# ZJU-FAST-Lab/Dftpav

Hardware: AMD Instinct MI355X
Metric: trajectory solves/sec (batched), 16-piece MINCO (higher is better)
Workload: dtype f64

## Files before the change

dftpav_amd/csrc/quad_common.h:

```cpp
#pragma once
#include "ref_order_common.h"

namespace dftpav {
namespace reford {

__device__ __forceinline__ double row_chain16(double acc, double v) {
  const double one = 1.0;
  asm volatile("s_nop 1\n\t" DFTPAV_FMAC_BCAST16 : "+v"(acc) : "v"(v), "v"(one));
  return acc;
}
__device__ __forceinline__ double row_add_lane0(double acc, double v) {
  const double one = 1.0;
  asm volatile("s_nop 1\n\t" DFTPAV_FMAC_BCAST(0) : "+v"(acc) : "v"(v), "v"(one));
  return acc;
}
__device__ __forceinline__ double row_max16(double v) {
  v = fmax(v, mov_dpp<0xB1>(v));
  v = fmax(v, mov_dpp<0x4E>(v));
  v = fmax(v, mov_dpp<0x141>(v));
  v = fmax(v, mov_dpp<0x140>(v));
  return v;
}
template <int CTRL> __device__ __forceinline__ double nb_dpp(double v) {
  int lo = __double2loint(v), hi = __double2hiint(v);
  lo = __builtin_amdgcn_update_dpp(0, lo, CTRL, 0xf, 0xf, true);
  hi = __builtin_amdgcn_update_dpp(0, hi, CTRL, 0xf, 0xf, true);
  return __hiloint2double(hi, lo);
}


constexpr int kQPool = 64;
__host__ __device__ constexpr size_t q4_team_doubles(int mem) { return 32 + 32 + 12 + 6 + sNUM + (size_t)mem + kQPool * 3 + kQPool / 8; }
__host__ __device__ constexpr size_t q4_team_bytes(int mem) { return (q4_team_doubles(mem) * sizeof(double) + iNUM * sizeof(int) + 15) & ~(size_t)15; }
__host__ __device__ constexpr size_t q4_shared_bytes(int N) { return ((size_t)pk_segment_doubles(N) * sizeof(double) + 15) & ~(size_t)15; }
constexpr size_t kDenseEntryBytes = 4 + 8 + 15 * 8;
__host__ __device__ constexpr size_t q4_dense_bytes_of(int k) { return ((size_t)k * kDenseEntryBytes + 15) & ~(size_t)15; }
constexpr int kDenseSizedForN = 16, kDenseSizedForMem = 256;
__host__ __device__ constexpr int q4_dense_capacity(int N, int mem) {
  int k = 64;
  while (k > 8 && 4 * (q4_shared_bytes(N) + 4 * q4_team_bytes(mem) + q4_dense_bytes_of(k)) > (size_t)160 * 1024) k -= 8;
  return k;
}
constexpr int kDense = q4_dense_capacity(kDenseSizedForN, kDenseSizedForMem);
static_assert(kDense % 8 == 0 && kDense >= 8 && kDense <= 64, "a lane's slots of the list are the bits of a 64-bit mask (solver_ref4.hip: mine |= 1ull << e)");
static_assert(4 * (q4_shared_bytes(kDenseSizedForN) + 4 * q4_team_bytes(kDenseSizedForMem) + q4_dense_bytes_of(kDense)) <= (size_t)160 * 1024,
              "four workgroups of one wave share a CU's LDS at 16 pieces and a history of 256");
typedef unsigned long long dmask_t;
struct DenseLds {
  ldsi_t id;
  ldsd_t s1;
  ldsd_t out;
};
__host__ __device__ constexpr size_t q4_dense_bytes() { return q4_dense_bytes_of(kDense); }
__device__ inline void q4_carve_dense(DenseLds &d, char *base) {
  ldsd_t p = (ldsd_t)reinterpret_cast<double *>(base);
  d.s1 = p; p += kDense;
  d.out = p; p += 15 * kDense;
  d.id = (ldsi_t)p;
}

}
}
```

dftpav_amd/csrc/solver_ref4.hip:

```cpp
#include <hip/hip_runtime.h>
#include <cstdio>
#include <cstdlib>
#include <algorithm>

#include "ref_order_common.h"
#include "quad_lbfgs.h"

namespace dftpav {
namespace reford {

static_assert(kQPool <= 64 && kQPool % 8 == 0, "a lane's pool slots are the bits of a 64-bit mask; the chain pass reads the permutation eight bytes at a time");
typedef unsigned char __attribute__((address_space(3))) *ldsb_t;
typedef const unsigned long long __attribute__((address_space(3))) *ldscu64_t;
#ifndef DFTPAV_Q4_WAVES_PER_EU
#define DFTPAV_Q4_WAVES_PER_EU 1
#endif
constexpr int kQ4WavesPerCU = 4 * DFTPAV_Q4_WAVES_PER_EU;

struct Q4 {
  ldsd_t xs, gs;
  ldsd_t bnd;
  ldsd_t tw;
  ldsd_t st;
  ldsd_t alpha;
  ldsd_t pool;
  ldsb_t perm;
  ldsi_t ist;
};
__device__ inline void q4_carve(Q4 &q, char *team, int mem) {
  ldsd_t p = (ldsd_t)reinterpret_cast<double *>(team);
  q.xs = p; p += 32;
  q.gs = p; p += 32;
  q.bnd = p; p += 12;
  q.tw = p; p += 6;
  q.st = p; p += sNUM;
  q.alpha = p; p += mem;
  q.pool = p; p += kQPool * 3;
  q.perm = (ldsb_t)p; p += kQPool / 8;
  q.ist = (ldsi_t)p;
}

__device__ __forceinline__ double row_sum32(double p0, double p1, int n, int l) {
  double acc = row_chain16(0.0, l < n ? p0 : -0.0);
  if (n > 16) acc = row_chain16(acc, 16 + l < n ? p1 : -0.0);
  return acc;
}
template <int Q>
__device__ __forceinline__ void sweep4(ldscd_t tab, double (&bq)[12], int N, int l) {
  constexpr bool DESC = Q == 1 || Q == 3, DIV = Q == 1 || Q == 2;
  ldscd_t ip = tab + 48;
  v2d_t c[pk_size(Q) / 2];
  {
    const int sl = DESC ? N - 1 - l : l;
    const int bi = sl >= 1 && sl <= N - 2 ? sl - 1 : 0;
    const ldscv2_t a = (ldscv2_t)(ip + bi * pk_size(Q));
    if (N > 2) {
#pragma unroll
      for (int u = 0; u < pk_size(Q) / 2; u++) c[u] = a[u];
    } else {
#pragma unroll
      for (int u = 0; u < pk_size(Q) / 2; u++) c[u] = v2d_t{0.0, 0.0};
    }
  }
#pragma unroll 1
  for (int s = 0; s < N; s++) {
    const int p = DESC ? N - 1 - s : s;
    double w[6][2];
#pragma unroll
    for (int r = 0; r < 6; r++)
#pragma unroll
      for (int d = 0; d < 2; d++) {
        w[r][d] = DESC ? nb_dpp<0x101>(bq[2 * (5 - r) + d]) : nb_dpp<0x111>(bq[2 * r + d]);
      }
    if (s == 0 || s == N - 1) {
      const ldscv2_t a = (ldscv2_t)(s == 0 ? tab : ip + (N - 2) * pk_size(Q));
      if (s == 0) {
#pragma unroll
        for (int r = 0; r < 6; r++) w[r][0] = w[r][1] = 0.0;
      }
      if (l == p) {
#pragma unroll
        for (int r = 0; r < 6; r++) {
          v2d_t ce[4];
#pragma unroll
          for (int u = 0; u < 4; u++) ce[u] = a[4 * r + u];
          const int rr = DESC ? 5 - r : r;
#pragma unroll
          for (int d = 0; d < 2; d++) {
            double acc = bq[2 * rr + d];
#pragma unroll
            for (int k = 0; k < 6; k++) {
              const double ck = (k & 1) ? ce[k >> 1].y : ce[k >> 1].x;
              const double t = ck * w[(r + k) % 6][d];
              acc = ck != 0.0 ? acc - t : acc;
            }
            if (DIV) acc = div_by_rcp(acc, ce[3].x, ce[3].y);
            w[r][d] = acc;
            bq[2 * rr + d] = acc;
          }
        }
      }
    } else {
      if (l == p) {
        auto at = [&](int o) { return (o & 1) ? c[o >> 1].y : c[o >> 1].x; };
#pragma unroll
        for (int r = 0; r < 6; r++) {
          const int rr = DESC ? 5 - r : r;
#pragma unroll
          for (int d = 0; d < 2; d++) {
            double acc = bq[2 * rr + d];
#pragma unroll
            for (int k = 0; k < 6; k++)
              if (pk_mask(Q, r) & (1 << k)) acc = acc - at(pk_off(Q, r, k)) * w[(r + k) % 6][d];
            if (DIV) acc = div_by_rcp(acc, at(pk_diag0(Q) + 2 * r), at(pk_diag0(Q) + 2 * r + 1));
            w[r][d] = acc;
            bq[2 * rr + d] = acc;
          }
        }
      }
    }
  }
}

__device__ __forceinline__ void q4_split(const double (&bq)[12], double (&X)[6], double (&Y)[6], int l) {
  const bool lo = (l & 8) == 0;
#pragma unroll
  for (int r = 0; r < 6; r++) {
    const double own = bq[2 * r], far = nb_dpp<0x128>(bq[2 * r + 1]);
    X[r] = lo ? own : far;
    Y[r] = lo ? far : own;
  }
}
__device__ __forceinline__ void q4_unsplit(const double (&X)[6], const double (&Y)[6], double (&bq)[12], int l) {
  const bool lo = (l & 8) == 0;
#pragma unroll
  for (int r = 0; r < 6; r++) {
    bq[2 * r] = lo ? X[r] : Y[r];
    bq[2 * r + 1] = nb_dpp<0x128>(lo ? Y[r] : X[r]);
  }
}
template <int Q>
__device__ __forceinline__ void sweep4_split(ldscd_t tab, double (&X)[6], double (&Y)[6], int l) {
  constexpr bool DESC = Q == 1 || Q == 3, DIV = Q == 1 || Q == 2;
  constexpr int N = 16;
  ldscd_t ip = tab + 48;
  const int l8 = l & 7;
  auto fetch = [&](const double (&R)[6], double (&w)[6]) {
#pragma unroll
    for (int r = 0; r < 6; r++) w[r] = DESC ? nb_dpp<0x101>(R[5 - r]) : nb_dpp<0x111>(R[r]);
  };
  auto end_step = [&](double (&R)[6], double (&w)[6], ldscv2_t a) {
    v2d_t cb[6][4];
#pragma unroll
    for (int r = 0; r < 6; r++)
#pragma unroll
      for (int u = 0; u < (DIV ? 4 : 3); u++) cb[r][u] = a[4 * r + u];
    asm volatile("" ::: "memory");
#pragma unroll
    for (int r = 0; r < 6; r++) {
      const v2d_t(&ce)[4] = cb[r];
      const int rr = DESC ? 5 - r : r;
      double acc = R[rr];
#pragma unroll
      for (int k = 0; k < 6; k++) {
        const double ck = (k & 1) ? ce[k >> 1].y : ce[k >> 1].x;
        const double t = ck * w[(r + k) % 6];
        acc = ck != 0.0 ? acc - t : acc;
      }
      if (DIV) acc = div_by_rcp(acc, ce[3].x, ce[3].y);
      w[r] = acc;
      R[rr] = acc;
    }
  };
  auto interior = [&](double (&R)[6], int s1, double (&w)[6]) {
    v2d_t c[pk_size(Q) / 2];
    {
      const int sl = (s1 & 8) + (DESC ? 7 - l8 : l8);
      const int bi = sl >= 1 && sl <= N - 2 ? sl - 1 : 0;
      const ldscv2_t a = (ldscv2_t)(ip + bi * pk_size(Q));
#pragma unroll
      for (int u = 0; u < pk_size(Q) / 2; u++) c[u] = a[u];
    }
    auto at = [&](int o) { return (o & 1) ? c[o >> 1].y : c[o >> 1].x; };
#pragma unroll 1
    for (int s = s1; s < s1 + 7; s++) {
      const bool own = l8 == ((DESC ? N - 1 - s : s) & 7);
      if (own) {
#pragma unroll
        for (int r = 0; r < 6; r++) {
          const int rr = DESC ? 5 - r : r;
          double acc = R[rr];
#pragma unroll
          for (int k = 0; k < 6; k++)
            if (pk_mask(Q, r) & (1 << k)) acc = acc - at(pk_off(Q, r, k)) * w[(r + k) % 6];
          if (DIV) acc = div_by_rcp(acc, at(pk_diag0(Q) + 2 * r), at(pk_diag0(Q) + 2 * r + 1));
          w[r] = acc;
          R[rr] = acc;
        }
      }
      fetch(R, w);
    }
  };
  double (&A)[6] = DESC ? Y : X;
  double (&B)[6] = DESC ? X : Y;
  double w[6] = {0.0, 0.0, 0.0, 0.0, 0.0, 0.0};
  if (l8 == (DESC ? 7 : 0)) end_step(A, w, (ldscv2_t)tab);
  fetch(A, w);
  interior(A, 1, w);
#pragma unroll
  for (int r = 0; r < 6; r++)
    w[r] = DESC ? nb_dpp<0x12F>(A[5 - r])
                : nb_dpp<0x121>(A[r]);
  interior(B, 8, w);
  if (l8 == (DESC ? 0 : 7)) end_step(B, w, (ldscv2_t)(ip + (N - 2) * pk_size(Q)));
}

struct RectSet {
  d2_t u[5];
};
__device__ __forceinline__ void load_rect(gcd2_t cor, RectSet &r) {
#pragma unroll
  for (int u = 0; u < 5; u++) r.u[u] = cor[16 * u];
}
__device__ __forceinline__ void rect_planes(const RectSet &r, double (&pl)[20]) {
  const double C = r.u[0].x, S = r.u[0].y;
  pl[0] = -S; pl[1] = C;
  pl[4] = C; pl[5] = S;
  pl[8] = S; pl[9] = -C;
  pl[12] = -C; pl[13] = -S;
#pragma unroll
  for (int k = 0; k < 4; k++) {
    pl[4 * k + 2] = r.u[1 + k].x;
    pl[4 * k + 3] = r.u[1 + k].y;
  }
#pragma unroll
  for (int u = 16; u < 20; u++) pl[u] = 0.0;
}
template <bool FAST, bool RECT>
__device__ __forceinline__ double q4_eval(const DevBatch &D, const Q4 &q, const DenseLds &dl, ldscd_t tab, gcd_t cor, size_t cpitch, gd_t ovf, int l, Prof &pr) {
  const DevLayout &L = D.L;
  const DevParams &P = D.P;
  const int N = L.Ntot, H = FAST ? 4 : L.H, nterm = 5 * H + 4, t0 = 5 * H;
  const double epis = FAST ? 0.0 : D.epis;
  const double vt = q.xs[L.x_tau0];
  const double Tr = vt > 0.0 ? ((0.5 * vt + 1.0) * vt + 1.0) + P.mini_T : 1.0 / ((0.5 * vt - 1.0) * vt + 1.0) + P.mini_T;
  const double t1 = Tr / N, t2 = t1 * t1, t3 = t2 * t1, t4 = t2 * t2, t5 = t4 * t1;
  pr.tick(10);
  double bq[12];
#pragma unroll
  for (int u = 0; u < 12; u++) bq[u] = 0.0;
  if (l == 0) {
#pragma unroll
    for (int d = 0; d < 2; d++) {
      bq[0 + d] = q.bnd[d];
      bq[2 + d] = q.bnd[2 + d] * t1;
      bq[4 + d] = q.bnd[4 + d] * t2;
    }
  }
  if (l == N - 1) {
#pragma unroll
    for (int d = 0; d < 2; d++) {
      bq[6 + d] = q.bnd[6 + d];
      bq[8 + d] = q.bnd[8 + d] * t1;
      bq[10 + d] = q.bnd[10 + d] * t2;
    }
  } else if (l < N - 1) {
    bq[10] = q.xs[2 * l];
    bq[11] = q.xs[2 * l + 1];
  }
  if (N == 16) {
    double X[6], Y[6];
    q4_split(bq, X, Y, l);
    sweep4_split<0>(tab, X, Y, l);
    sweep4_split<1>(tab + pk_sweep_offset(1, 16), X, Y, l);
    q4_unsplit(X, Y, bq, l);
  } else {
    sweep4<0>(tab, bq, N, l);
    sweep4<1>(tab + pk_sweep_offset(1, N), bq, N, l);
  }
  pr.tick(0);
  double cc[12];
  {
    const double tI[6] = {1.0 / 1.0, 1.0 / t1, 1.0 / t2, 1.0 / t3, 1.0 / t4, 1.0 / t5};
#pragma unroll
    for (int u = 0; u < 12; u++) cc[u] = bq[u] * tI[u >> 1];
    if (l == 0) {
#pragma unroll
      for (int u = 0; u < 6; u++) q.tw[u] = tI[u];
    }
  }
  double gdC[12], pE, pG;
  {
    const double *c = cc;
    const double t[6] = {1.0, t1, t2, t3, t4, t5};
    const double n33 = c[6] * c[6] + c[7] * c[7], n44 = c[8] * c[8] + c[9] * c[9], n55 = c[10] * c[10] + c[11] * c[11];
    const double d43 = c[8] * c[6] + c[9] * c[7], d53 = c[10] * c[6] + c[11] * c[7], d54 = c[10] * c[8] + c[11] * c[9];
    pE = 36.0 * n33 * t[1] + 144.0 * d43 * t[2] + 192.0 * n44 * t[3] + 240.0 * d53 * t[3] + 720.0 * d54 * t[4] + 720.0 * n55 * t[5];
    pG = 36.0 * n33 + 288.0 * d43 * t[1] + 576.0 * n44 * t[2] + 720.0 * d53 * t[2] + 2880.0 * d54 * t[3] + 3600.0 * n55 * t[4];
#pragma unroll
    for (int d = 0; d < 2; d++) {
      const double c3 = c[6 + d], c4 = c[8 + d], c5 = c[10 + d];
      gdC[10 + d] = 240.0 * c3 * t[3] + 720.0 * c4 * t[4] + 1440.0 * c5 * t[5];
      gdC[8 + d] = 144.0 * c3 * t[2] + 384.0 * c4 * t[3] + 720.0 * c5 * t[4];
      gdC[6 + d] = 72.0 * c3 * t[1] + 144.0 * c4 * t[2] + 240.0 * c5 * t[3];
      gdC[d] = 0.0;
      gdC[2 + d] = 0.0;
      gdC[4 + d] = 0.0;
    }
  }
  pr.tick(1);
  const bool piece = l < N;
  const int Kl = (l == 0 || l == N - 1) ? L.Kd : L.K;
  const int pt0 = l == 0 ? 0 : (L.Kd + 1) + (l - 1) * (L.K + 1);
  const double step = t1 / Kl;
  const int singul_ = L.singuls[0];
  double s1 = 0.0;
  int cnt = 0;
  int rcnt = 0;
  unsigned long long pmask = 0ull;
  const gd_t ovf_l = ovf + (size_t)pt0 * nterm * 3;
  double pl[20];
  RectSet rs;
  const gcd2_t rcor = (gcd2_t)cor;
  if constexpr (RECT) load_rect(rcor, rs);
  else load_planes(cor, cpitch, H, pl);
  __builtin_amdgcn_s_waitcnt(0x0F70);
  auto take = [&](const double (&r12)[12], double e0, double e1, double e2, int slot) {
#pragma unroll
    for (int u = 0; u < 12; u++) gdC[u] += r12[u];
    if (slot < kQPool) {
      ldsd_t e = q.pool + slot * 3;
      e[0] = e0;
      e[1] = e1;
      e[2] = e2;
      pmask |= 1ull << slot;
    } else {
      gd_t e = ovf_l + (size_t)cnt * 3;
      e[0] = e0;
      e[1] = e1;
      e[2] = e2;
    }
    cnt++;
  };
  const int lane64 = (int)(threadIdx.x & 63);
  int listed = 0;
  dmask_t mine = 0ull;
  const unsigned long long here = __builtin_amdgcn_ballot_w64(true);
  const int row_here[4] = {(int)(here & 1ull), (int)((here >> 16) & 1ull), (int)((here >> 32) & 1ull), (int)((here >> 48) & 1ull)};
  const int my_row = lane64 >> 4;
  const int rank = ((my_row > 0 ? row_here[0] : 0) + (my_row > 1 ? row_here[1] : 0) + (my_row > 2 ? row_here[2] : 0)) * 16 + l;
  const int n_here = 16 * (row_here[0] + row_here[1] + row_here[2] + row_here[3]);
  auto scan_here = [&](int c, int &total, int &row_incl) {
    int v = c;
    v += __builtin_amdgcn_update_dpp(0, v, 0x111, 0xf, 0xf, false);
    v += __builtin_amdgcn_update_dpp(0, v, 0x112, 0xf, 0xf, false);
    v += __builtin_amdgcn_update_dpp(0, v, 0x114, 0xf, 0xf, false);
    v += __builtin_amdgcn_update_dpp(0, v, 0x118, 0xf, 0xf, false);
    row_incl = v;
    const int t0_ = row_here[0] ? __builtin_amdgcn_readlane(v, 15) : 0, t1_ = row_here[1] ? __builtin_amdgcn_readlane(v, 31) : 0;
    const int t2_ = row_here[2] ? __builtin_amdgcn_readlane(v, 47) : 0, t3_ = row_here[3] ? __builtin_amdgcn_readlane(v, 63) : 0;
    total = t0_ + t1_ + t2_ + t3_;
    return v + (my_row > 0 ? t0_ : 0) + (my_row > 1 ? t1_ : 0) + (my_row > 2 ? t2_ : 0);
  };
  auto flush = [&]() {
    for (int first = 0; first < listed; first += n_here) {
    const int slot = first + rank;
    const bool work = slot < listed;
    const int id = dl.id[work ? slot : 0];
    const int o = id & 63, t = (id >> 6) & 63, jo = id >> 12;
    double cco[12];
#pragma unroll
    for (int u = 0; u < 12; u++) cco[u] = __shfl(cc[u], o);
    const double t1o = __shfl(t1, o);
    const int lo = o & 15;
    const int Ko = (lo == 0 || lo == N - 1) ? L.Kd : L.K;
    const double stepo = t1o / Ko;
    if (work) {
      const double nopl[20] = {0.0, 0.0, 0.0, 0.0, 0.0, 0.0, 0.0, 0.0, 0.0, 0.0, 0.0, 0.0, 0.0, 0.0, 0.0, 0.0, 0.0, 0.0, 0.0, 0.0};
      PtState ps;
      (void)point_masks<false>(P, cco, lo, N, jo, Ko, stepo, dl.s1[slot], singul_, epis, H, nopl, (gd_t) nullptr, D.sur, 0.0, 0.0, 0, 0.0, ps);
      double r_[16];
      ldsd_t w = dl.out + 15 * slot;
      const double pk[4] = {w[0], w[1], w[2], w[3]};
      point_emit_pf(P, ps, t, H, t0, [&](int, double &on0, double &on1, double &q0, double &q1) { on0 = pk[0]; on1 = pk[1]; q0 = pk[2]; q1 = pk[3]; },
                    (double *)r_);
      const bool corr = t < t0;
#pragma unroll
      for (int u = 0; u < 13; u++) w[u] = r_[u];
      w[13] = corr ? r_[13] : -0.0;
      w[14] = corr ? -0.0 : r_[13];
    }
    }
    __builtin_amdgcn_fence(__ATOMIC_SEQ_CST, "wavefront");
    unsigned rlo = (unsigned)mine, rhi = (unsigned)(mine >> 32);
    rlo |= (unsigned)__builtin_amdgcn_update_dpp(0, (int)rlo, 0x121, 0xf, 0xf, false);
    rhi |= (unsigned)__builtin_amdgcn_update_dpp(0, (int)rhi, 0x121, 0xf, 0xf, false);
    rlo |= (unsigned)__builtin_amdgcn_update_dpp(0, (int)rlo, 0x122, 0xf, 0xf, false);
    rhi |= (unsigned)__builtin_amdgcn_update_dpp(0, (int)rhi, 0x122, 0xf, 0xf, false);
    rlo |= (unsigned)__builtin_amdgcn_update_dpp(0, (int)rlo, 0x124, 0xf, 0xf, false);
    rhi |= (unsigned)__builtin_amdgcn_update_dpp(0, (int)rhi, 0x124, 0xf, 0xf, false);
    rlo |= (unsigned)__builtin_amdgcn_update_dpp(0, (int)rlo, 0x128, 0xf, 0xf, false);
    rhi |= (unsigned)__builtin_amdgcn_update_dpp(0, (int)rhi, 0x128, 0xf, 0xf, false);
    const dmask_t rowm = ((dmask_t)rhi << 32) | rlo;
    for (dmask_t mm = mine; mm;) {
      const int i = __builtin_ctzll(mm);
      mm &= mm - 1;
      ldscd_t w = dl.out + 15 * i;
      double r12[12];
#pragma unroll
      for (int u = 0; u < 12; u++) r12[u] = w[u];
      take(r12, w[12], w[13], w[14], rcnt + __builtin_popcountll(rowm & ((1ull << i) - 1ull)));
    }
    rcnt += __builtin_popcountll(rowm);
    __builtin_amdgcn_fence(__ATOMIC_SEQ_CST, "wavefront");
    listed = 0;
    mine = 0ull;
  };
#pragma unroll 1
  for (int j = 0; j <= L.Kmax + 1; j++) {
    const bool extra = j > L.Kmax;
    unsigned m = 0u;
    PtState pst;
    double nx[20];
    RectSet nr;
    if constexpr (RECT) {
      load_rect(rcor + (size_t)(j < L.Kmax ? j + 1 : L.Kmax) * 80, nr);
      rect_planes(rs, pl);
    } else {
      load_planes(cor + (size_t)(j < L.Kmax ? j + 1 : L.Kmax) * 16, cpitch, H, nx);
    }
    if (piece && j <= Kl && !extra)
      m = (unsigned)point_masks<false>(P, cc, l, N, j, Kl, step, s1, singul_, epis, H, pl, (gd_t) nullptr, D.sur, 0.0, 0.0, 0, 0.0, pst);
    const double s1_pt = s1;
    s1 += step;
    [[maybe_unused]] long long emit_t0 = 0;
    if (D.prof != nullptr) {
#if defined(DFTPAV_PROF_EMIT_CYCLES)
      emit_t0 = clock64();
#elif defined(DFTPAV_PROF_FLUSH_CYCLES)
#else
      const int pc = __builtin_popcount(m);
      int trips = 0;
      while (__builtin_amdgcn_ballot_w64(pc > trips) != 0ull) trips++;
      pr.count(11, trips);
#endif
    }
    auto plane_of = [&](int k, double &on0, double &on1, double &q0, double &q1) {
      on0 = pl[0]; on1 = pl[1]; q0 = pl[2]; q1 = pl[3];
#pragma unroll
      for (int u = 1; u < 5; u++) {
        on0 = k == u ? pl[4 * u] : on0;
        on1 = k == u ? pl[4 * u + 1] : on1;
        q0 = k == u ? pl[4 * u + 2] : q0;
        q1 = k == u ? pl[4 * u + 3] : q1;
      }
    };
    bool in_place = false;
    const int c = __builtin_popcount(m);
    const bool any = __builtin_amdgcn_ballot_w64(c != 0) != 0ull;
    int incl = 0, total = 0, row_incl = 0;
    if (any) incl = scan_here(c, total, row_incl);
    if (listed > 0 && (extra || listed + total > kDense)) {
#ifdef DFTPAV_PROF_FLUSH_CYCLES
      const long long flush_t0 = D.prof != nullptr ? clock64() : 0;
#endif
      flush();
      if (D.prof != nullptr) {
        pr.count(9, 1ll << 32);
#ifdef DFTPAV_PROF_FLUSH_CYCLES
        pr.count(11, clock64() - flush_t0);
#endif
      }
    }
    if (any && total > kDense) {
      in_place = true;
    } else if (any) {
      int e = listed + incl - c;
      for (unsigned mm = m; mm;) {
        const int t = __builtin_ctz(mm);
        mm &= mm - 1;
        dl.id[e] = lane64 | (t << 6) | (j << 12);
        dl.s1[e] = s1_pt;
        if (t < t0) {
          int v = 0;
#pragma unroll
          for (int qv = 1; qv < 5; qv++) v += t >= qv * H ? 1 : 0;
          double on0, on1, q0, q1;
          plane_of(t - v * H, on0, on1, q0, q1);
          ldsd_t w = dl.out + 15 * e;
          w[0] = on0;
          w[1] = on1;
          w[2] = q0;
          w[3] = q1;
        }
        mine |= 1ull << e;
        e++;
      }
      listed += total;
    }
    if (in_place) {
      int slot = rcnt + row_incl - c;
      rcnt += __builtin_amdgcn_update_dpp(0, row_incl, 0x15F, 0xf, 0xf, false);
      for (unsigned mm = m; mm;) {
        const int t = __builtin_ctz(mm);
        mm &= mm - 1;
        double r_[16];
        point_emit_pf(P, pst, t, H, t0, plane_of, (double *)r_);
        const bool corr = t < t0;
        double r12[12];
#pragma unroll
        for (int u = 0; u < 12; u++) r12[u] = r_[u];
        take(r12, r_[12], corr ? r_[13] : -0.0, corr ? -0.0 : r_[13], slot++);
      }
    }
#ifdef DFTPAV_PROF_EMIT_CYCLES
    if (D.prof != nullptr) pr.count(11, clock64() - emit_t0);
#endif
    if constexpr (RECT) {
      rs = nr;
    } else {
#pragma unroll
      for (int u = 0; u < 20; u++) pl[u] = nx[u];
    }
  }
  __threadfence_block();
  pr.tick(2);
  double gdT = row_chain16(0.0, piece ? pG : -0.0);
  const double en = row_chain16(0.0, piece ? pE : -0.0);
  double cost0 = 0.0, cost2 = 0.0;
  {
    const int pc = piece ? cnt : 0;
    int incl = pc;
    incl += __builtin_amdgcn_update_dpp(0, incl, 0x111, 0xf, 0xf, false);
    incl += __builtin_amdgcn_update_dpp(0, incl, 0x112, 0xf, 0xf, false);
    incl += __builtin_amdgcn_update_dpp(0, incl, 0x114, 0xf, 0xf, false);
    incl += __builtin_amdgcn_update_dpp(0, incl, 0x118, 0xf, 0xf, false);
    const int total = __builtin_amdgcn_update_dpp(0, incl, 0x15F, 0xf, 0xf, false);
    pr.count(9, total);
    int kmax = 0;
#pragma unroll
    for (int r = 0; r < 4; r++)
      if (row_here[r]) kmax = max(kmax, __builtin_amdgcn_readlane(incl, 16 * r + 15));
    const bool slow = kmax > kQPool;
    if (D.prof != nullptr) pr.count(11, slow ? 1ll << 32 : 0ll);
    if (kmax > 0 && !slow) {
      {
        int at = incl - pc;
        for (unsigned long long mm = pmask; mm;) {
          q.perm[at++] = (unsigned char)__builtin_ctzll(mm);
          mm &= mm - 1;
        }
      }
      __builtin_amdgcn_fence(__ATOMIC_SEQ_CST, "wavefront");
      for (int k0 = 0; k0 < kmax; k0 += 8) {
        const unsigned long long pb = *(ldscu64_t)(q.perm + k0);
        double e[8][3];
#pragma unroll
        for (int u = 0; u < 8; u++) {
          const int sl = k0 + u < total ? (int)((pb >> (8 * u)) & 255ull) : 0;
#pragma unroll
          for (int w = 0; w < 3; w++) e[u][w] = q.pool[sl * 3 + w];
        }
#pragma unroll
        for (int u = 0; u < 8; u++) {
          const bool in = k0 + u < total;
          gdT += in ? e[u][0] : -0.0;
          cost0 += in ? e[u][1] : -0.0;
          cost2 += in ? e[u][2] : -0.0;
        }
      }
    } else if (slow) {
      for (int p = 0; p < N; p++) {
        const int src = (lane64 & 48) | p;
        const int c = __shfl(pc, src);
        if (__builtin_amdgcn_ballot_w64(c != 0) == 0ull) continue;
        const unsigned long long pm = ((unsigned long long)(unsigned)__shfl((int)(pmask >> 32), src) << 32) | (unsigned)__shfl((int)pmask, src);
        for (unsigned long long mm = pm; mm;) {
          ldscd_t e = q.pool + __builtin_ctzll(mm) * 3;
          mm &= mm - 1;
          gdT += e[0];
          cost0 += e[1];
          cost2 += e[2];
        }
        const int pp0 = p == 0 ? 0 : (L.Kd + 1) + (p - 1) * (L.K + 1);
        const gcd_t og = (gcd_t)(ovf + (size_t)pp0 * nterm * 3);
        for (int i0 = __builtin_popcountll(pm); i0 < c; i0 += 8) {
          double e[8][3];
#pragma unroll
          for (int u = 0; u < 8; u++) {
            const int i = i0 + u < c ? i0 + u : c - 1;
#pragma unroll
            for (int w = 0; w < 3; w++) e[u][w] = og[(size_t)i * 3 + w];
          }
#pragma unroll
          for (int u = 0; u < 8; u++) {
            if (i0 + u < c) {
              gdT += e[u][0];
              cost0 += e[u][1];
              cost2 += e[u][2];
            }
          }
        }
      }
    }
  }
  pr.tick(3);
  double pA;
  double tI[6];
#pragma unroll
  for (int u = 0; u < 6; u++) tI[u] = q.tw[u];
  {
    const double gdtInv[6] = {0.0, -1.0 * tI[2], -2.0 * tI[3], -3.0 * tI[4], -4.0 * tI[5], -5.0 * tI[5] * tI[1]};
    double acc = 0.0;
#pragma unroll
    for (int k = 0; k < 6; k++) {
      const double gdcol = gdC[2 * k] * bq[2 * k] + gdC[2 * k + 1] * bq[2 * k + 1];
      acc += gdtInv[k] * gdcol;
    }
    pA = acc;
  }
  double adj[12];
#pragma unroll
  for (int u = 0; u < 12; u++) adj[u] = gdC[u] * tI[u >> 1];
  if (N == 16) {
    double X[6], Y[6];
    q4_split(adj, X, Y, l);
    sweep4_split<2>(tab + pk_sweep_offset(2, 16), X, Y, l);
    sweep4_split<3>(tab + pk_sweep_offset(3, 16), X, Y, l);
    q4_unsplit(X, Y, adj, l);
  } else {
    sweep4<2>(tab + pk_sweep_offset(2, N), adj, N, l);
    sweep4<3>(tab + pk_sweep_offset(3, N), adj, N, l);
  }
  pr.tick(4);
  if (l < N - 1) {
    q.gs[2 * l] = adj[10];
    q.gs[2 * l + 1] = adj[11];
  }
  {
    double hv[6], tv[6];
#pragma unroll
    for (int u = 0; u < 6; u++) {
      hv[u] = q.bnd[u];
      tv[u] = q.bnd[6 + u];
    }
    const double h1 = hv[2] * adj[2] + hv[3] * adj[3];
    const double h2 = (hv[4] * adj[4] + hv[5] * adj[5]) * 2.0 * t1;
    const double g1 = tv[2] * adj[8] + tv[3] * adj[9];
    const double g2 = (tv[4] * adj[10] + tv[5] * adj[11]) * 2.0 * t1;
    gdT = row_add_lane0(gdT, h1);
    gdT = row_add_lane0(gdT, h2);
    gdT = row_chain16(gdT, l == N - 1 ? g1 : -0.0);
    gdT = row_chain16(gdT, l == N - 1 ? g2 : -0.0);
    gdT = row_chain16(gdT, piece ? pA : -0.0);
    double gdVT2Rt;
    if (vt > 0) {
      gdVT2Rt = vt + 1.0;
    } else {
      const double denSqrt = (0.5 * vt - 1.0) * vt + 1.0;
      gdVT2Rt = (1.0 - vt) / (denSqrt * denSqrt);
    }
    if (l == 0) q.gs[L.x_tau0] = (gdT / N + P.wei_time) * gdVT2Rt;
  }
  double total_smcost = 0.0, total_timecost = 0.0, penalty_cost = 0.0;
  total_smcost += en;
  penalty_cost += (cost0 + 0.0) + cost2;
  total_timecost += Tr * P.wei_time;
  __builtin_amdgcn_fence(__ATOMIC_SEQ_CST, "wavefront");
  pr.tick(5);
  return total_smcost + total_timecost + penalty_cost;
}


constexpr int kQB = 8;
constexpr int kQNpad = 64;
static_assert(kQuadMirrorRows == 2 * kQB, "DevBatch::histM holds kQB rows of either end of a ring");
template <bool Y3> struct QBlk {
  d2_t a[kQB], b[kQB];
  d2_t yr[Y3 ? kQB : 1];
};
typedef double __attribute__((ext_vector_type(2))) qd2_t;

#define DFTPAV_FMAC_BCAST15 \
  DFTPAV_FMAC_BCAST(0) DFTPAV_FMAC_BCAST(1) DFTPAV_FMAC_BCAST(2) DFTPAV_FMAC_BCAST(3) DFTPAV_FMAC_BCAST(4) DFTPAV_FMAC_BCAST(5) DFTPAV_FMAC_BCAST(6) \
  DFTPAV_FMAC_BCAST(7) DFTPAV_FMAC_BCAST(8) DFTPAV_FMAC_BCAST(9) DFTPAV_FMAC_BCAST(10) DFTPAV_FMAC_BCAST(11) DFTPAV_FMAC_BCAST(12) \
  DFTPAV_FMAC_BCAST(13) DFTPAV_FMAC_BCAST(14)
__device__ __forceinline__ double row_chain15(double acc, double v) {
  const double one = 1.0;
  asm volatile("s_nop 1\n\t" DFTPAV_FMAC_BCAST15 : "+v"(acc) : "v"(v), "v"(one));
  return acc;
}
template <bool Y3> __device__ __forceinline__ double q4_rec_sum(double p0, double p1, int n) {
  double acc = row_chain16(0.0, p0);
  if (n > 16) acc = Y3 ? row_chain16(acc, p1) : row_chain15(acc, p1);
  return acc;
}

template <int DIR, bool Y3>
__device__ __forceinline__ void q4_load_blk(QBlk<Y3> &R, gcd2_t hS, gcd2_t hM, gcd2_t hR, int m, int l, int &jl) {
  const bool wrap = DIR < 0 ? jl < kQB - 1 : jl > m - kQB;
  const int mr = DIR < 0 ? kQB + jl : jl - (m - kQB);
  const gcd2_t row = (wrap ? hM + mr * kQNpad : hS + jl * kQNpad) + l;
#pragma unroll
  for (int u = 0; u < kQB; u++) {
    R.a[u] = row[DIR * u * kQNpad];
    R.b[u] = row[DIR * u * kQNpad + 16];
  }
  if (Y3) {
    int jr = jl;
#pragma unroll
    for (int u = 0; u < kQB; u++) {
      R.yr[Y3 ? u : 0] = hR[jr];
      if (DIR < 0) jr = jr == 0 ? m - 1 : jr - 1;
      else jr = jr == m - 1 ? 0 : jr + 1;
    }
  }
  if (DIR < 0) {
    jl -= kQB;
    jl = jl < 0 ? jl + m : jl;
  } else {
    jl += kQB;
    jl = jl >= m ? jl - m : jl;
  }
}
template <bool Y3> __device__ __forceinline__ void q4_pin_blk(QBlk<Y3> &R) {
#pragma unroll
  for (int u = 0; u < kQB; u++) {
    asm volatile("" : "+v"(R.a[u].x), "+v"(R.a[u].y), "+v"(R.b[u].x), "+v"(R.b[u].y));
    if (Y3) asm volatile("" : "+v"(R.yr[Y3 ? u : 0].x), "+v"(R.yr[Y3 ? u : 0].y));
  }
}
template <bool Y3> __device__ __forceinline__ d2_t q4_blk_yr(const QBlk<Y3> &R, int u) {
  if (Y3) return R.yr[Y3 ? u : 0];
  d2_t yr;
  yr.x = mov_dpp<0x15F>(R.b[u].x);
  yr.y = mov_dpp<0x15F>(R.b[u].y);
  return yr;
}
template <bool EXACT, bool Y3>
__device__ __forceinline__ void q4_first_steps(const QBlk<Y3> &R, ldsd_t al, int i0, int bound, int n, int l, bool exact, double &d0, double &d1) {
#pragma unroll
  for (int u = 0; u < kQB; u++) {
    if (i0 + u < bound) {
      const d2_t yr = q4_blk_yr<Y3>(R, u);
      const double dot = q4_rec_sum<Y3>(R.a[u].x * d0, R.b[u].x * d1, n);
      const double a = EXACT && exact ? dot / yr.x : div_by_rcp<false>(dot, yr.x, yr.y);
      if (l == 0) al[u] = a;
      const double na = -a;
      d0 = d0 + na * R.a[u].y;
      d1 = d1 + na * R.b[u].y;
    }
  }
}
template <bool EXACT, bool Y3>
__device__ __forceinline__ void q4_second_steps(const QBlk<Y3> &R, ldscd_t al, int i0, int bound, int n, int l, bool exact, double &d0, double &d1) {
#pragma unroll
  for (int u = 0; u < kQB; u++) {
    if (i0 + u < bound) {
      const double av = al[kQB - 1 - u];
      const d2_t yr = q4_blk_yr<Y3>(R, u);
      const double dot = q4_rec_sum<Y3>(R.a[u].y * d0, R.b[u].y * d1, n);
      const double beta = EXACT && exact ? dot / yr.x : div_by_rcp<false>(dot, yr.x, yr.y);
      const double cf = av - beta;
      d0 = d0 + cf * R.a[u].x;
      d1 = d1 + cf * R.b[u].x;
    }
  }
}
template <bool EXACT, bool Y3>
__device__ __forceinline__ void q4_two_loop(const Q4 &q, gcd2_t hS, gcd2_t hM, gcd2_t hR, int m, int n, int l, int bound, int ne, bool exact, double sc0, double &d0,
                                            double &d1) {
  QBlk<Y3> A, B;
  int jl = ne == 0 ? m - 1 : ne - 1;
  q4_load_blk<-1>(A, hS, hM, hR, m, l, jl);
#pragma unroll 1
  for (int i0 = 0; i0 < bound; i0 += 2 * kQB) {
    q4_pin_blk(A);
    q4_load_blk<-1>(B, hS, hM, hR, m, l, jl);
    q4_first_steps<EXACT>(A, q.alpha + i0, i0, bound, n, l, exact, d0, d1);
    q4_pin_blk(B);
    q4_load_blk<-1>(A, hS, hM, hR, m, l, jl);
    q4_first_steps<EXACT>(B, q.alpha + (i0 + kQB), i0 + kQB, bound, n, l, exact, d0, d1);
  }
  d0 = d0 * sc0;
  d1 = d1 * sc0;
  __builtin_amdgcn_fence(__ATOMIC_SEQ_CST, "wavefront");
  jl = ne - bound;
  jl = jl < 0 ? jl + m : jl;
  q4_load_blk<+1>(A, hS, hM, hR, m, l, jl);
#pragma unroll 1
  for (int i0 = 0; i0 < bound; i0 += 2 * kQB) {
    const ldscd_t al = (ldscd_t)(q.alpha + (bound - kQB - i0));
    q4_pin_blk(A);
    q4_load_blk<+1>(B, hS, hM, hR, m, l, jl);
    q4_second_steps<EXACT>(A, al, i0, bound, n, l, exact, d0, d1);
    q4_pin_blk(B);
    q4_load_blk<+1>(A, hS, hM, hR, m, l, jl);
    q4_second_steps<EXACT>(B, al - kQB, i0 + kQB, bound, n, l, exact, d0, d1);
  }
}
__device__ __forceinline__ void q4_store_pair(gd_t hS, gd_t hM, int m, int end, int e, d2_t v) {
  ((gd2_t)hS)[(size_t)end * kQNpad + e] = v;
  if (end < kQB) ((gd2_t)hM)[(kQB + end) * kQNpad + e] = v;
  if (end >= m - kQB) ((gd2_t)hM)[(end - (m - kQB)) * kQNpad + e] = v;
}

struct Q4Shape {
  static constexpr int NV = 2;
  typedef Q4 Row;
  gd_t hS, hM, hR;
  __device__ __forceinline__ double row_sum(const double (&p)[2], int n, int l) const { return row_sum32(p[0], p[1], n, l); }
  __device__ __forceinline__ void store_pair(int m, int end, int e, d2_t sy) const { q4_store_pair(hS, hM, m, end, e, sy); }
  __device__ __forceinline__ void store_ys(int m, int end, int n, int l, d2_t yr) const {
    if (l == 0) ((gd2_t)hR)[end] = yr;
    if (l == 15 && n <= 31) q4_store_pair(hS, hM, m, end, 31, yr);
  }
  template <bool EXACT>
  __device__ __forceinline__ void two_loop(const Q4 &q, int m, int n, int l, int bound, int ne, bool exact, double sc0, double (&d)[2]) const {
    const gcd2_t cS = (gcd2_t)hS, cM = (gcd2_t)hM, cR = (gcd2_t)hR;
    if (n > 31) q4_two_loop<EXACT, true>(q, cS, cM, cR, m, n, l, bound, ne, exact, sc0, d[0], d[1]);
    else q4_two_loop<EXACT, false>(q, cS, cM, cR, m, n, l, bound, ne, exact, sc0, d[0], d[1]);
  }
};

template <bool FAST, bool RECT>
__global__ void __launch_bounds__(256, DFTPAV_Q4_WAVES_PER_EU)
    ref4_kernel(const DevBatch *__restrict__ Dp, int mode, const double *__restrict__ tabs, const double *__restrict__ cor_t, double *__restrict__ scratch, int source,
                int slice, int hand) {
  extern __shared__ double lds_raw[];
  const DevBatch &D = *Dp;
  const DevLayout &L = D.L;
  const int tidb = threadIdx.x, Tb = blockDim.x, lane = tidb & 63, wv = tidb >> 6, W = Tb >> 6, row = lane >> 4, l = lane & 15;
  const int n = L.n, N = L.Ntot, H = L.H, mem = D.P.mem_size;
  Q4 q;
  q4_carve(q, reinterpret_cast<char *>(lds_raw) + q4_shared_bytes(N) + (size_t)(wv * 4 + row) * q4_team_bytes(mem), mem);
  DenseLds dl;
  q4_carve_dense(dl, reinterpret_cast<char *>(lds_raw) + q4_shared_bytes(N) + (size_t)W * 4 * q4_team_bytes(mem) + (size_t)wv * q4_dense_bytes());
  const ldscd_t tab = (ldscd_t)lds_raw;
  for (int i = tidb; i < pk_segment_doubles(N); i += Tb) ((ldsd_t)lds_raw)[i] = tabs[i];
  __syncthreads();
  const bool ring = mode == kModeSolve && (source & 1) != 0;
  const bool force_exact_div = (source & 2) != 0;
  const int nterm = 5 * H + 4, JP = L.Kmax + 1;
  const size_t cpitch = (size_t)JP * 16;
  const size_t scratch_per_traj = (size_t)L.Npts * nterm * kRec + (size_t)L.Npts * nterm;
  Prof pr;
  pr.on = false;
  pr.acc = nullptr;
  pr.last = 0;
  QuadVec<2> v{};
  QuadRun r{-1, false, false, 0};
  int steps = 0;

  for (int pass = 0;; pass++) {
    if (!r.act && quad_take(D, q, v, r, mode, ring, force_exact_div, pass, pr)) {
      if (l < 12) q.bnd[l] = l < 6 ? D.iniS[(size_t)r.b * 6 + l] : D.finS[(size_t)r.b * 6 + (l - 6)];
      __builtin_amdgcn_fence(__ATOMIC_SEQ_CST, "wavefront");
    }
    if (__builtin_amdgcn_ballot_w64(r.act) == 0ull) break;
    if (r.act) {
      const int b = r.b;
      const gcd_t cor = RECT ? (gcd_t)(cor_t + ((size_t)b * JP * 80 + l) * 2) : (gcd_t)(cor_t + (size_t)b * L.H * 4 * cpitch + l);
      const gd_t ovf = (gd_t)(scratch + (size_t)b * scratch_per_traj);
      const double f = q4_eval<FAST, RECT>(D, q, dl, tab, cor, cpitch, ovf, l, pr);
      if (mode == kModeEval) {
        for (int h = 0; h < 2; h++) {
          const int e = 16 * h + l;
          if (e < n) D.g_out[(size_t)b * n + e] = q.gs[e];
        }
        if (l == 0) D.f_eval[b] = f;
        r.act = false;
      } else {
        const Q4Shape sh{(gd_t)(D.histS + (size_t)b * mem * kQNpad * 2), (gd_t)(D.histM + (size_t)b * kQuadMirrorRows * kQNpad * 2),
                         (gd_t)(D.histR + (size_t)b * mem * 2)};
        quad_advance(D, sh, q, v, f, l, pr);
        __builtin_amdgcn_fence(__ATOMIC_SEQ_CST, "wavefront");
        if (q.ist[iACTION] == kActDone) quad_results<2>(D, q, r, ring);
      }
    }
    if (!ring) {
      if (mode == kModeEval) break;
      continue;
    }
    steps++;
    if (slice > 0 && steps >= slice) {
      steps = 0;
      if (quad_end_slice(D, q, v, r, hand)) break;
    }
  }
}

__global__ void q4_corridor_kernel(const double *__restrict__ cor, double *__restrict__ out, int B, int H4, int NptsPad, int N, int K, int Kd, int JP) {
  const size_t total = (size_t)B * H4 * JP * 16;
  for (size_t i = (size_t)blockIdx.x * blockDim.x + threadIdx.x; i < total; i += (size_t)gridDim.x * blockDim.x) {
    const int p = (int)(i & 15);
    const size_t r = i >> 4;
    const int j = (int)(r % JP);
    const size_t bc = r / JP;
    double v = 0.0;
    if (p < N) {
      const int Kp = (p == 0 || p == N - 1) ? Kd : K;
      const int pt0 = p == 0 ? 0 : (Kd + 1) + (p - 1) * (K + 1);
      if (j <= Kp) v = cor[bc * NptsPad + pt0 + j];
    }
    out[i] = v;
  }
}

__global__ void q4_rect_check_kernel(const double *__restrict__ cor, int B, int Npts, int NptsPad, int *__restrict__ flag) {
  const size_t total = (size_t)B * Npts;
  const unsigned long long sign = 0x8000000000000000ull;
  for (size_t i = (size_t)blockIdx.x * blockDim.x + threadIdx.x; i < total; i += (size_t)gridDim.x * blockDim.x) {
    const size_t b = i / Npts;
    const int pt = (int)(i % Npts);
    const double *c = cor + b * 16 * NptsPad + pt;
    unsigned long long n[4][2];
    for (int k = 0; k < 4; k++)
      for (int q = 0; q < 2; q++) n[k][q] = (unsigned long long)__double_as_longlong(c[(size_t)(4 * k + q) * NptsPad]);
    const unsigned long long C = n[1][0], S = n[1][1];
    const bool nan = (C & ~sign) > 0x7ff0000000000000ull || (S & ~sign) > 0x7ff0000000000000ull;
    const bool ok = !nan && n[0][0] == (S ^ sign) && n[0][1] == C && n[2][0] == S && n[2][1] == (C ^ sign) && n[3][0] == (C ^ sign) && n[3][1] == (S ^ sign);
    if (!ok) *flag = 1;
  }
}

__global__ void q4_corridor_rect_kernel(const double *__restrict__ cor, d2_t *__restrict__ out, int B, int NptsPad, int N, int K, int Kd, int JP) {
  const size_t total = (size_t)B * JP * 80;
  for (size_t i = (size_t)blockIdx.x * blockDim.x + threadIdx.x; i < total; i += (size_t)gridDim.x * blockDim.x) {
    const int p = (int)(i & 15);
    const int u = (int)((i >> 4) % 5);
    const size_t r = i / 80;
    const int j = (int)(r % JP);
    const size_t b = r / JP;
    d2_t v = {0.0, 0.0};
    if (p < N) {
      const int Kp = (p == 0 || p == N - 1) ? Kd : K;
      const int pt0 = p == 0 ? 0 : (Kd + 1) + (p - 1) * (K + 1);
      if (j <= Kp) {
        const int c0 = u == 0 ? 4 : 4 * (u - 1) + 2;
        const double *src = cor + (b * 16 + c0) * NptsPad + pt0 + j;
        v.x = src[0];
        v.y = src[NptsPad];
      }
    }
    out[i] = v;
  }
}

}

bool reference_order_quad_supported(const DevLayout &L, const DevParams &P, int S) {
  if (L.M != 1 || S != 0 || L.n > 32 || L.Ntot > 16 || L.Ntot < 2 || L.H < 1 || L.H > 5) return false;
  if (L.npad != reford::kQNpad || P.mem_size < reford::kQB) return false;
  return reford::q4_shared_bytes(L.Ntot) + 4 * reford::q4_team_bytes(P.mem_size) + reford::q4_dense_bytes() <= 160 * 1024;
}
extern "C" int dftpav_debug_quad_list_capacity(void) { return reford::kDense; }
size_t reference_order_quad_corridor_doubles(const DevLayout &L, int B) { return (size_t)B * L.H * 4 * (L.Kmax + 1) * 16; }
QuadSizes reference_order_quad_sizes(const DevLayout &L, const DevParams &P) {
  return {reford::q4_shared_bytes(L.Ntot), reford::q4_team_bytes(P.mem_size) + (reford::q4_dense_bytes() + 3) / 4, reford::kQ4WavesPerCU, 768};
}
hipError_t launch_quad_corridor(const DevBatch &D, double *cor_t, bool rect, hipStream_t stream) {
  const DevLayout &L = D.L;
  const size_t total = rect ? (size_t)D.B * (L.Kmax + 1) * 80 : reference_order_quad_corridor_doubles(L, D.B);
  const int grid = (int)std::min<size_t>((total + 255) / 256, 65536);
  if (rect)
    hipLaunchKernelGGL(reford::q4_corridor_rect_kernel, dim3(grid), dim3(256), 0, stream, D.corridor, reinterpret_cast<reford::d2_t *>(cor_t), D.B, D.NptsPad, L.Ntot, L.K,
                       L.Kd, L.Kmax + 1);
  else
    hipLaunchKernelGGL(reford::q4_corridor_kernel, dim3(grid), dim3(256), 0, stream, D.corridor, cor_t, D.B, L.H * 4, D.NptsPad, L.Ntot, L.K, L.Kd, L.Kmax + 1);
  return hipGetLastError();
}
hipError_t launch_quad_rect_check(const double *corridor, int B, int Npts, int NptsPad, int *d_flag, hipStream_t stream) {
  hipError_t e = hipMemsetAsync(d_flag, 0, sizeof(int), stream);
  if (e != hipSuccess) return e;
  const size_t total = (size_t)B * Npts;
  const int grid = (int)std::min<size_t>((total + 255) / 256, 65536);
  hipLaunchKernelGGL(reford::q4_rect_check_kernel, dim3(grid), dim3(256), 0, stream, corridor, B, Npts, NptsPad, d_flag);
  return hipGetLastError();
}
QuadKernel ref4_kernel_for(bool fast, bool rect) {
  if (fast && rect) return &reford::ref4_kernel<true, true>;
  return fast ? &reford::ref4_kernel<true, false> : &reford::ref4_kernel<false, false>;
}

}
```

Baseline: 46220.

## Route overflowing pool entries through the chain pass with 16-bit scratch codes

```diff
diff --git a/dftpav_amd/csrc/quad_common.h b/dftpav_amd/csrc/quad_common.h
--- a/dftpav_amd/csrc/quad_common.h
+++ b/dftpav_amd/csrc/quad_common.h
@@ -30,12 +30,23 @@
 
 
 constexpr int kQPool = 64;
-__host__ __device__ constexpr size_t q4_team_doubles(int mem) { return 32 + 32 + 12 + 6 + sNUM + (size_t)mem + kQPool * 3 + kQPool / 8; }
-__host__ __device__ constexpr size_t q4_team_bytes(int mem) { return (q4_team_doubles(mem) * sizeof(double) + iNUM * sizeof(int) + 15) & ~(size_t)15; }
+__host__ __device__ constexpr size_t q4_team_doubles_of(int mem, int chain) { return 32 + 32 + 12 + 6 + sNUM + (size_t)mem + kQPool * 3 + (size_t)chain / 4; }
+__host__ __device__ constexpr size_t q4_team_bytes_of(int mem, int chain) {
+  return (q4_team_doubles_of(mem, chain) * sizeof(double) + iNUM * sizeof(int) + 15) & ~(size_t)15;
+}
 __host__ __device__ constexpr size_t q4_shared_bytes(int N) { return ((size_t)pk_segment_doubles(N) * sizeof(double) + 15) & ~(size_t)15; }
 constexpr size_t kDenseEntryBytes = 4 + 8 + 15 * 8;
 __host__ __device__ constexpr size_t q4_dense_bytes_of(int k) { return ((size_t)k * kDenseEntryBytes + 15) & ~(size_t)15; }
 constexpr int kDenseSizedForN = 16, kDenseSizedForMem = 256;
+__host__ __device__ constexpr int q4_chain_capacity(int N, int mem) {
+  int k = kQPool;
+  while (4 * (q4_shared_bytes(N) + 4 * q4_team_bytes_of(mem, k + 8) + q4_dense_bytes_of(64)) <= (size_t)160 * 1024) k += 8;
+  return k;
+}
+constexpr int kQChain = q4_chain_capacity(kDenseSizedForN, kDenseSizedForMem);
+static_assert(kQChain % 8 == 0 && kQChain >= kQPool && kQChain <= 1024, "codes are read eight at a time; a row within its pool needs kQPool of them");
+__host__ __device__ constexpr size_t q4_team_doubles(int mem) { return q4_team_doubles_of(mem, kQChain); }
+__host__ __device__ constexpr size_t q4_team_bytes(int mem) { return q4_team_bytes_of(mem, kQChain); }
 __host__ __device__ constexpr int q4_dense_capacity(int N, int mem) {
   int k = 64;
   while (k > 8 && 4 * (q4_shared_bytes(N) + 4 * q4_team_bytes(mem) + q4_dense_bytes_of(k)) > (size_t)160 * 1024) k -= 8;
@@ -43,6 +54,7 @@
 }
 constexpr int kDense = q4_dense_capacity(kDenseSizedForN, kDenseSizedForMem);
 static_assert(kDense % 8 == 0 && kDense >= 8 && kDense <= 64, "a lane's slots of the list are the bits of a 64-bit mask (solver_ref4.hip: mine |= 1ull << e)");
+static_assert(kDense == 64, "the permutation table is sized beside a full list: it must not shorten it");
 static_assert(4 * (q4_shared_bytes(kDenseSizedForN) + 4 * q4_team_bytes(kDenseSizedForMem) + q4_dense_bytes_of(kDense)) <= (size_t)160 * 1024,
               "four workgroups of one wave share a CU's LDS at 16 pieces and a history of 256");
 typedef unsigned long long dmask_t;
diff --git a/dftpav_amd/csrc/solver_ref4.hip b/dftpav_amd/csrc/solver_ref4.hip
--- a/dftpav_amd/csrc/solver_ref4.hip
+++ b/dftpav_amd/csrc/solver_ref4.hip
@@ -9,8 +9,15 @@
 namespace dftpav {
 namespace reford {
 
-static_assert(kQPool <= 64 && kQPool % 8 == 0, "a lane's pool slots are the bits of a 64-bit mask; the chain pass reads the permutation eight bytes at a time");
-typedef unsigned char __attribute__((address_space(3))) *ldsb_t;
+static_assert(kQPool <= 64 && kQPool % 8 == 0, "a lane's pool slots are the bits of a 64-bit mask");
+constexpr unsigned kQCodeScratch = 0x8000u;
+constexpr int kQCodeEntries = 1024;
+static_assert(kQPool <= (int)kQCodeScratch && 15 << 10 < (int)kQCodeScratch, "a pool slot and a piece's number fit a code");
+__host__ __device__ constexpr unsigned q4_scratch_code(int piece, int i) { return kQCodeScratch | (unsigned)(piece << 10) | (unsigned)i; }
+__host__ __device__ constexpr bool q4_code_is_scratch(unsigned code) { return (code & kQCodeScratch) != 0u; }
+__host__ __device__ constexpr int q4_code_piece(unsigned code) { return (int)((code >> 10) & 15u); }
+__host__ __device__ constexpr int q4_code_entry(unsigned code) { return (int)(code & (unsigned)(kQCodeEntries - 1)); }
+typedef unsigned short __attribute__((address_space(3))) *ldsh_t;
 typedef const unsigned long long __attribute__((address_space(3))) *ldscu64_t;
 #ifndef DFTPAV_Q4_WAVES_PER_EU
 #define DFTPAV_Q4_WAVES_PER_EU 1
@@ -24,7 +31,7 @@
   ldsd_t st;
   ldsd_t alpha;
   ldsd_t pool;
-  ldsb_t perm;
+  ldsh_t perm;
   ldsi_t ist;
 };
 __device__ inline void q4_carve(Q4 &q, char *team, int mem) {
@@ -36,7 +43,7 @@
   q.st = p; p += sNUM;
   q.alpha = p; p += mem;
   q.pool = p; p += kQPool * 3;
-  q.perm = (ldsb_t)p; p += kQPool / 8;
+  q.perm = (ldsh_t)p; p += kQChain / 4;
   q.ist = (ldsi_t)p;
 }
 
@@ -149,13 +156,14 @@
 #pragma unroll
     for (int r = 0; r < 6; r++) w[r] = DESC ? nb_dpp<0x101>(R[5 - r]) : nb_dpp<0x111>(R[r]);
   };
-  auto end_step = [&](double (&R)[6], double (&w)[6], ldscv2_t a) {
-    v2d_t cb[6][4];
+  auto end_rows = [&](v2d_t (&cb)[6][4], ldscv2_t a) {
 #pragma unroll
     for (int r = 0; r < 6; r++)
 #pragma unroll
       for (int u = 0; u < (DIV ? 4 : 3); u++) cb[r][u] = a[4 * r + u];
     asm volatile("" ::: "memory");
+  };
+  auto end_step = [&](double (&R)[6], double (&w)[6], const v2d_t (&cb)[6][4]) {
 #pragma unroll
     for (int r = 0; r < 6; r++) {
       const v2d_t(&ce)[4] = cb[r];
@@ -185,18 +193,16 @@
 #pragma unroll 1
     for (int s = s1; s < s1 + 7; s++) {
       const bool own = l8 == ((DESC ? N - 1 - s : s) & 7);
-      if (own) {
-#pragma unroll
-        for (int r = 0; r < 6; r++) {
-          const int rr = DESC ? 5 - r : r;
-          double acc = R[rr];
-#pragma unroll
-          for (int k = 0; k < 6; k++)
-            if (pk_mask(Q, r) & (1 << k)) acc = acc - at(pk_off(Q, r, k)) * w[(r + k) % 6];
-          if (DIV) acc = div_by_rcp(acc, at(pk_diag0(Q) + 2 * r), at(pk_diag0(Q) + 2 * r + 1));
-          w[r] = acc;
-          R[rr] = acc;
-        }
+#pragma unroll
+      for (int r = 0; r < 6; r++) {
+        const int rr = DESC ? 5 - r : r;
+        double acc = R[rr];
+#pragma unroll
+        for (int k = 0; k < 6; k++)
+          if (pk_mask(Q, r) & (1 << k)) acc = acc - at(pk_off(Q, r, k)) * w[(r + k) % 6];
+        if (DIV) acc = div_by_rcp(acc, at(pk_diag0(Q) + 2 * r), at(pk_diag0(Q) + 2 * r + 1));
+        w[r] = acc;
+        R[rr] = own ? acc : R[rr];
       }
       fetch(R, w);
     }
@@ -204,15 +210,20 @@
   double (&A)[6] = DESC ? Y : X;
   double (&B)[6] = DESC ? X : Y;
   double w[6] = {0.0, 0.0, 0.0, 0.0, 0.0, 0.0};
-  if (l8 == (DESC ? 7 : 0)) end_step(A, w, (ldscv2_t)tab);
+  v2d_t cb[6][4];
+  if (l8 == (DESC ? 7 : 0)) {
+    end_rows(cb, (ldscv2_t)tab);
+    end_step(A, w, cb);
+  }
   fetch(A, w);
   interior(A, 1, w);
 #pragma unroll
   for (int r = 0; r < 6; r++)
     w[r] = DESC ? nb_dpp<0x12F>(A[5 - r])
                 : nb_dpp<0x121>(A[r]);
+  end_rows(cb, (ldscv2_t)(ip + (N - 2) * pk_size(Q)));
   interior(B, 8, w);
-  if (l8 == (DESC ? 0 : 7)) end_step(B, w, (ldscv2_t)(ip + (N - 2) * pk_size(Q)));
+  if (l8 == (DESC ? 0 : 7)) end_step(B, w, cb);
 }
 
 struct RectSet {
@@ -438,6 +449,7 @@
 #if defined(DFTPAV_PROF_EMIT_CYCLES)
       emit_t0 = clock64();
 #elif defined(DFTPAV_PROF_FLUSH_CYCLES)
+#elif defined(DFTPAV_PROF_CHAIN_CYCLES)
 #else
       const int pc = __builtin_popcount(m);
       int trips = 0;
@@ -542,24 +554,53 @@
     for (int r = 0; r < 4; r++)
       if (row_here[r]) kmax = max(kmax, __builtin_amdgcn_readlane(incl, 16 * r + 15));
     const bool slow = kmax > kQPool;
-    if (D.prof != nullptr) pr.count(11, slow ? 1ll << 32 : 0ll);
-    if (kmax > 0 && !slow) {
+    const bool piecewise = slow && (kmax > kQChain || nterm * (L.Kmax + 1) > kQCodeEntries);
+    if (D.prof != nullptr) pr.count(11, (slow ? 1ll << 32 : 0ll) + (piecewise ? 1ll << 48 : 0ll));
+    if (kmax > 0 && !piecewise) {
       {
         int at = incl - pc;
         for (unsigned long long mm = pmask; mm;) {
-          q.perm[at++] = (unsigned char)__builtin_ctzll(mm);
+          q.perm[at++] = (unsigned short)__builtin_ctzll(mm);
           mm &= mm - 1;
         }
+        for (int i = __builtin_popcountll(pmask); i < pc; i++) q.perm[at++] = (unsigned short)q4_scratch_code(l, i);
       }
       __builtin_amdgcn_fence(__ATOMIC_SEQ_CST, "wavefront");
+      const gcd_t og = (gcd_t)ovf;
       for (int k0 = 0; k0 < kmax; k0 += 8) {
-        const unsigned long long pb = *(ldscu64_t)(q.perm + k0);
+        const ldscu64_t pp = (ldscu64_t)(q.perm + k0);
+        const unsigned long long pb_lo = pp[0], pb_hi = pp[1];
+        unsigned code[8], anyc = 0u;
+#pragma unroll
+        for (int u = 0; u < 8; u++) {
+          const unsigned cw = (unsigned)(((u < 4 ? pb_lo : pb_hi) >> (16 * (u & 3))) & 0xffffull);
+          code[u] = k0 + u < total ? cw : 0u;
+          anyc |= code[u];
+        }
         double e[8][3];
 #pragma unroll
         for (int u = 0; u < 8; u++) {
-          const int sl = k0 + u < total ? (int)((pb >> (8 * u)) & 255ull) : 0;
+          const int sl = q4_code_is_scratch(code[u]) ? 0 : (int)code[u];
 #pragma unroll
           for (int w = 0; w < 3; w++) e[u][w] = q.pool[sl * 3 + w];
+        }
+        if (slow && __builtin_amdgcn_ballot_w64(q4_code_is_scratch(anyc)) != 0ull) {
+          double ge[8][3];
+#pragma unroll
+          for (int u = 0; u < 8; u++) {
+            const bool g = q4_code_is_scratch(code[u]);
+            const int p = q4_code_piece(code[u]), i = q4_code_entry(code[u]);
+            const int pp0 = p == 0 ? 0 : (L.Kd + 1) + (p - 1) * (L.K + 1);
+            const int off = g ? (pp0 * nterm + i) * 3 : 0;
+#pragma unroll
+            for (int w = 0; w < 3; w++) ge[u][w] = og[off + w];
+          }
+#pragma unroll
+          for (int u = 0; u < 8; u++) {
+            const bool g = q4_code_is_scratch(code[u]);
+#pragma unroll
+            for (int w = 0; w < 3; w++) e[u][w] = g ? ge[u][w] : e[u][w];
+          }
         }
 #pragma unroll
         for (int u = 0; u < 8; u++) {
@@ -569,7 +610,7 @@
           cost2 += in ? e[u][2] : -0.0;
         }
       }
-    } else if (slow) {
+    } else if (piecewise) {
       for (int p = 0; p < N; p++) {
         const int src = (lane64 & 48) | p;
         const int c = __shfl(pc, src);
@@ -603,6 +644,9 @@
         }
       }
     }
+#ifdef DFTPAV_PROF_CHAIN_CYCLES
+    if (D.prof != nullptr && slow) pr.count(11, clock64() - pr.last);
+#endif
   }
   pr.tick(3);
   double pA;
@@ -955,6 +999,15 @@
   return reford::q4_shared_bytes(L.Ntot) + 4 * reford::q4_team_bytes(P.mem_size) + reford::q4_dense_bytes() <= 160 * 1024;
 }
 extern "C" int dftpav_debug_quad_list_capacity(void) { return reford::kDense; }
+extern "C" int dftpav_debug_quad_chain_capacity(void) { return reford::kQChain; }
+extern "C" int dftpav_debug_quad_chain_code(int piece, int i, int *out ) {
+  if (piece < 0 || piece > 15 || i < 0 || i >= reford::kQCodeEntries || out == nullptr) return -1;
+  const unsigned code = reford::q4_scratch_code(piece, i);
+  out[0] = reford::q4_code_is_scratch(code) ? 1 : 0;
+  out[1] = reford::q4_code_piece(code);
+  out[2] = reford::q4_code_entry(code);
+  return (int)code;
+}
 size_t reference_order_quad_corridor_doubles(const DevLayout &L, int B) { return (size_t)B * L.H * 4 * (L.Kmax + 1) * 16; }
 QuadSizes reference_order_quad_sizes(const DevLayout &L, const DevParams &P) {
   return {reford::q4_shared_bytes(L.Ntot), reford::q4_team_bytes(P.mem_size) + (reford::q4_dense_bytes() + 3) / 4, reford::kQ4WavesPerCU, 768};
```

After: 46810 (median of 6 runs). +1.3%, better.
